# zkonduit/ezkl

Measured on NVIDIA H100. Metric: prove_time_s, lower is better.
Workload: dtype u32 limbs (254-bit Montgomery integers mod BN254 r/p)

## Files before the change

### ezkl_b200/csrc/debug.cu

```cuda
#include "../../include/ezkl_b200.h"
#include <cfenv>
#include <vector>
#include "msm.cuh"
#include "../../tools/experiments/fd.cuh"
#include "../../tools/experiments/msm_affine.cuh"

namespace b200 {
template <class Tag>
__global__ void k_dbg_field(int op, const Fp<Tag>* a, const Fp<Tag>* b, Fp<Tag>* o, size_t n) {
    size_t i = (size_t)blockIdx.x * blockDim.x + threadIdx.x;
    if (i >= n) return;
    Fp<Tag> x = fp_load(a + i), y = fp_load(b + i), r;
    if (op == 0) r = x + y; else if (op == 1) r = x - y; else if (op == 2) r = x * y; else if (op == 3) r = fp_inv(x); else r = fp_from_mont(x);
    fp_store(o + i, r);
}
__global__ void k_dbg_g1(int op, const G1Affine* a, const G1Affine* b, G1Affine* o, size_t n) {
    size_t i = (size_t)blockIdx.x * blockDim.x + threadIdx.x;
    if (i >= n) return;
    G1Affine p = a[i], q = b[i];
    G1Xyzz r;
    if (op == 0) r = g1_add_mixed(g1_to_xyzz(p), q);
    else if (op == 1) r = g1_dbl(g1_to_xyzz(p));
    else if (op == 2) r = g1_mul_small(g1_to_xyzz(p), q.x.l[0]);
    else if (op == 3) r = g1_add(g1_to_xyzz(p), g1_dbl_affine(q));
// ... 165 lines not shown
    for (size_t i = 0; i < n_ents; ++i) if ((ents[i] & 0x7fffffffu) + 1 > n_pts) n_pts = (ents[i] & 0x7fffffffu) + 1;
    tab.resize(n_pts);
    memcpy(tab.data(), table, 64 * n_pts);
    int rc = b200::msm_affine_host_chunks(tab.data(), ents, n_ents, chunk_start, chunk_len, nchunks, res.data());
    memcpy(out, res.data(), 64 * nchunks);
    return rc;
}
int b200_debug_bench(int variant, int iters, int blocks, int threads, float* ms) {
    Fq* d; B200_CUDA(cudaMalloc(&d, sizeof(Fq) * (size_t)blocks * threads));
    cudaEvent_t e0, e1; cudaEventCreate(&e0); cudaEventCreate(&e1);
    for (int rep = 0; rep < 2; ++rep) {
        cudaEventRecord(e0);
        switch (variant) {
            case 0: k_bench_mul<0><<<blocks, threads>>>(d, iters); break;
            case 1: k_bench_mul<1><<<blocks, threads>>>(d, iters); break;
            case 2: k_bench_mul<2><<<blocks, threads>>>(d, iters); break;
            case 3: k_bench_mul<3><<<blocks, threads>>>(d, iters); break;
            case 10: k_bench_hybrid<0><<<blocks, threads>>>(d, iters); break;
            case 11: k_bench_hybrid<1><<<blocks, threads>>>(d, iters); break;
            case 12: k_bench_hybrid<2><<<blocks, threads>>>(d, iters); break;
            case 13: k_bench_hybrid<3><<<blocks, threads>>>(d, iters); break;
            case 14: k_bench_hybrid<4><<<blocks, threads>>>(d, iters); break;
            case 15: k_bench_hybrid<5><<<blocks, threads>>>(d, iters); break;
            case 16: k_bench_hybrid<6><<<blocks, threads>>>(d, iters); break;
            case 17: k_bench_hybrid<7><<<blocks, threads>>>(d, iters); break;
            case 18: k_bench_hybrid<8><<<blocks, threads>>>(d, iters); break;
            default: k_bench_mul<4><<<blocks, threads>>>(d, iters); break;
        }
        cudaEventRecord(e1);
        B200_CUDA(cudaEventSynchronize(e1));
    }
    B200_CUDA(cudaEventElapsedTime(ms, e0, e1));
    cudaFree(d); cudaEventDestroy(e0); cudaEventDestroy(e1);
    return 0;
}
int b200_debug_bench_pipe(int variant, int iters, int blocks, int threads, float* ms) {
    uint64_t* d; B200_CUDA(cudaMalloc(&d, 8 * (size_t)blocks * threads));
    cudaEvent_t e0, e1; cudaEventCreate(&e0); cudaEventCreate(&e1);
    for (int rep = 0; rep < 2; ++rep) {
        cudaEventRecord(e0);
        switch (variant) {
            case 0: k_bench_pipe<0><<<blocks, threads>>>(d, iters); break;
            case 1: k_bench_pipe<1><<<blocks, threads>>>(d, iters); break;
            case 2: k_bench_pipe<2><<<blocks, threads>>>(d, iters); break;
            default: k_bench_pipe<3><<<blocks, threads>>>(d, iters); break;
        }
        cudaEventRecord(e1);
        B200_CUDA(cudaEventSynchronize(e1));
    }
    B200_CUDA(cudaEventElapsedTime(ms, e0, e1));
    cudaFree(d); cudaEventDestroy(e0); cudaEventDestroy(e1);
    return 0;
}
int b200_debug_digits_host(const b200_fr* s_canonical, size_t n, int c, int32_t* out) {
    const int W = (255 + c - 1) / c;
    for (size_t i = 0; i < n; ++i) {
        uint32_t v[8]; memcpy(v, &s_canonical[i], 32);
        uint32_t carry = 0;
        for (int w = 0; w < W; ++w) out[i * W + w] = msm_next_digit(v, c, &carry);
    }
    return 0;
}
int b200_debug_digit_slots_host(const b200_fr* s_canonical, size_t n, int c, int wpl, int32_t* out) {
    const int W = (255 + c - 1) / c;
    for (size_t i = 0; i < n; ++i) {
        uint32_t v[8]; memcpy(v, &s_canonical[i], 32);
        uint32_t carry = 0;
        MsmWindowSlot slot;
        for (int w = 0; w < W; ++w) {
            const int32_t d = msm_next_digit(v, c, &carry);
            int32_t* o = out + ((size_t)i * W + w) * 4;
            o[0] = (int32_t)slot.level; o[1] = slot.r;
            o[2] = d ? (int32_t)(slot.set_off + (uint32_t)(d < 0 ? -d : d) - 1u) : -1;
            o[3] = d < 0 ? -1 : (d > 0 ? 1 : 0);
            slot.next(c, wpl);
        }
    }
    return 0;
}
int b200_debug_msm_pick_levels(size_t n, int c, size_t max_table_bytes, int* s, int* L) {
    msm_pick_levels(n, c, max_table_bytes, s, L);
    return 0;
}
int b200_debug_host_g1_op(int op, const b200_g1_affine* a, const b200_g1_affine* b, b200_g1_affine* out, size_t n) {
    for (size_t i = 0; i < n; ++i) {
        G1Affine p, q; memcpy(&p, &a[i], 64); memcpy(&q, &b[i], 64);
        G1Xyzz r;
        if (op == 0) r = g1_add_mixed(g1_to_xyzz(p), q);
        else if (op == 1) r = g1_dbl(g1_to_xyzz(p));
        else if (op == 2) r = g1_mul_small(g1_to_xyzz(p), q.x.l[0]);
        else if (op == 3) r = g1_add(g1_to_xyzz(p), g1_dbl_affine(q));
        else r = g1_add_mixed(g1_to_xyzz(p), g1_neg(p));
        G1Affine o = g1_to_affine(r); memcpy(&out[i], &o, 64);
    }
    return 0;
}
int b200_debug_host_field_op(int field, int op, const b200_fr* a, const b200_fr* b, b200_fr* out, size_t n) {
    for (size_t i = 0; i < n; ++i) {
        if (field == 0) { Fr x, y, r; memcpy(&x, &a[i], 32); memcpy(&y, &b[i], 32);
            if (op == 0) r = x + y; else if (op == 1) r = x - y; else if (op == 2) r = x * y; else if (op == 3) r = fp_inv(x); else r = fp_from_mont(x);
            memcpy(&out[i], &r, 32);
        } else { Fq x, y, r; memcpy(&x, &a[i], 32); memcpy(&y, &b[i], 32);
            if (op == 0) r = x + y; else if (op == 1) r = x - y; else if (op == 2) r = x * y; else if (op == 3) r = fp_inv(x); else r = fp_from_mont(x);
            memcpy(&out[i], &r, 32);
        }
    }
    return 0;
}
}
#pragma GCC visibility pop
```

### ezkl_b200/csrc/msm.cu

```cuda
#include "msm.cuh"
#include "ec_coop.cuh"

namespace b200 {

static constexpr int HEAVY_CHUNKS = 32;
static constexpr int REDUCE_M_MAX = 32;
static constexpr int TREE_THREADS = 256;

int msm_default_window(size_t n) {
    int k = 0;
    while (((size_t)1 << (k + 1)) <= n) ++k;
    int c = k <= 10 ? 8 : (k <= 13 ? k - 2 : (k <= 17 ? k - 1 : (k <= 19 ? 17 : (k <= 21 ? 18 : 20))));
    if (c < 4) c = 4;
    if (c > 22) c = 22;
    return c;
}

__global__ void __launch_bounds__(128) k_table_next_level(const G1Affine* __restrict__ prev, G1Affine* __restrict__ next, size_t n, int c) {
    size_t i = (size_t)blockIdx.x * blockDim.x + threadIdx.x;
    if (i >= n) return;
    G1Affine p = prev[i];
    G1Xyzz a = g1_dbl_affine(p);
#pragma unroll 1
    for (int j = 1; j < c; ++j) a = g1_dbl(a);
    next[i] = g1_to_affine(a);
}

int msm_table_alloc(MsmTable* t, size_t n, int c, size_t max_table_bytes) {
    B200_CHECK(n > 0, -1, "msm_table_build: empty base vector");
    if (c <= 0) c = msm_default_window(n);
    int W = (255 + c - 1) / c, s = 1, L = W;
    msm_pick_levels(n, c, max_table_bytes, &s, &L);
    B200_CHECK((size_t)L * n < ((size_t)1 << 31), -1, "msm_table_build: L*n = %zu exceeds the 31-bit entry index", (size_t)L * n);
    t->n = n; t->c = c; t->W = W; t->s = s; t->L = L;
    B200_CUDA(cudaGetDevice(&t->device));
    const cudaError_t e = cudaMalloc(&t->d_table, t->bytes());
    if (e != cudaSuccess) {
        cudaGetLastError();
        t->d_table = nullptr;
        set_error("msm_table_build: %zu MiB table (%d levels of %zu points): %s", t->bytes() >> 20, L, n, cudaGetErrorString(e));
        return -2;
    }
    return 0;
}

int msm_table_build(MsmTable* t, const G1Affine* d_bases, cudaStream_t st) {
    const size_t n = t->n;
    if (d_bases) B200_CUDA(cudaMemcpyAsync(t->d_table, d_bases, sizeof(G1Affine) * n, cudaMemcpyDeviceToDevice, st));
    for (int j = 1; j < t->L; ++j) {
        k_table_next_level<<<div_up(n, 128), 128, 0, st>>>(t->d_table + (size_t)(j - 1) * n, t->d_table + (size_t)j * n, n, t->c * t->s); count_launch();
    }
    B200_CUDA(cudaGetLastError());
    return 0;
}
void msm_table_free(MsmTable* t) {
    if (t->d_table) cudaFree(t->d_table);
    t->d_table = nullptr;
}

template <bool SCATTER, bool SUBWIN>
__global__ void __launch_bounds__(256) k_digits(const Fr* __restrict__ scalars, size_t stride, uint32_t n, uint32_t table_n, uint32_t base_off, int c, int W,
                                                 uint32_t nbuckets, uint32_t* __restrict__ counters ,
                                                 const uint32_t* __restrict__ offs , uint32_t* __restrict__ ents, size_t ent_stride,
                                                 const uint32_t* __restrict__ skew, int wpl) {
    const uint32_t col = blockIdx.y;
    const bool aggregate = !SCATTER || skew[col] != 0;
    const Fr* sc = scalars + (size_t)col * stride;
    uint32_t* cnt = counters + (size_t)col * nbuckets;
    const uint32_t* off = SCATTER ? offs + (size_t)col * (nbuckets + 1) : nullptr;
    uint32_t* ent = SCATTER ? ents + (size_t)col * ent_stride : nullptr;
    const unsigned lane = threadIdx.x & 31;
    const uint32_t n_up = (n + 31u) & ~31u;
    for (uint32_t i = blockIdx.x * blockDim.x + threadIdx.x; i < n_up; i += gridDim.x * blockDim.x) {
        const bool valid = i < n;
        Fr s = fp_zero<FrTag>();
        if (valid) s = fp_from_mont(fp_load(sc + i));
        uint32_t carry = 0;
        MsmWindowSlot slot;
#pragma unroll 1
        for (int w = 0; w < W; ++w) {
            int32_t d = msm_next_digit(s.l, c, &carry);
            const uint32_t j = SUBWIN ? slot.level : (uint32_t)w;
            const bool nz = d != 0;
            const unsigned act = __ballot_sync(0xffffffffu, nz);
            if (nz && !aggregate) {
                const uint32_t bucket = (SUBWIN ? slot.set_off : 0u) + (uint32_t)(d < 0 ? -d : d) - 1u;
                ent[off[bucket] + atomicAdd(&cnt[bucket], 1u)] = (j * table_n + base_off + i) | (d < 0 ? 0x80000000u : 0u);
            } else if (nz) {
                const uint32_t bucket = (SUBWIN ? slot.set_off : 0u) + (uint32_t)(d < 0 ? -d : d) - 1u;
                const unsigned peers = __match_any_sync(act, bucket);
                const int leader = __ffs(peers) - 1;
                uint32_t base = 0;
                if ((int)lane == leader) base = atomicAdd(&cnt[bucket], (uint32_t)__popc(peers));
                if (SCATTER) {
                    base = __shfl_sync(peers, base, leader);
                    const uint32_t rank = __popc(peers & ((1u << lane) - 1u));
                    ent[off[bucket] + base + rank] = (j * table_n + base_off + i) | (d < 0 ? 0x80000000u : 0u);
                }
            }
            if (SUBWIN) slot.next(c, wpl);
        }
    }
}

__global__ void __launch_bounds__(1024) k_scan_buckets(const uint32_t* __restrict__ counts, uint32_t* __restrict__ offs, uint32_t* __restrict__ chunk_offs,
                                                        uint32_t nbuckets, uint32_t cap, uint32_t* __restrict__ skew ) {
    __shared__ uint32_t sh_max;
    if (threadIdx.x == 0) sh_max = 0;
    __syncthreads();
    const uint32_t col = blockIdx.x;
    const uint32_t lc = 31u - (uint32_t)__clz(cap);
    const uint32_t* cnt = counts + (size_t)col * nbuckets;
    uint32_t* off = offs + (size_t)col * (nbuckets + 1);
    uint32_t* coff = chunk_offs + (size_t)col * (nbuckets + 1);
    const uint32_t ipt = (nbuckets + blockDim.x - 1) / blockDim.x;
    const uint32_t lo = threadIdx.x * ipt, hi = min(lo + ipt, nbuckets);
    uint32_t s = 0, cs = 0;
    uint32_t mx = 0;
    const bool vec = (ipt & 3u) == 0 && lo + ipt <= nbuckets;
    if (vec) {
        const uint4* c4 = reinterpret_cast<const uint4*>(cnt + lo);
#pragma unroll 4
        for (uint32_t q = 0; q < (ipt >> 2); ++q) {
            const uint4 v = c4[q];
            s += v.x + v.y + v.z + v.w;
            cs += ((v.x + cap - 1) >> lc) + ((v.y + cap - 1) >> lc) + ((v.z + cap - 1) >> lc) + ((v.w + cap - 1) >> lc);
            mx = max(max(mx, v.x), max(max(v.y, v.z), v.w));
        }
    } else {
        for (uint32_t b = lo; b < hi; ++b) { uint32_t v = cnt[b]; s += v; cs += ((v + cap - 1) >> lc); mx = max(mx, v); }
    }
    if (mx) atomicMax(&sh_max, mx);
    uint32_t tot, ctot;
    uint32_t ex = block_exclusive_scan(s, &tot);
    uint32_t cex = block_exclusive_scan(cs, &ctot);
    if (vec) {
        const uint4* c4 = reinterpret_cast<const uint4*>(cnt + lo);
#pragma unroll 4
        for (uint32_t q = 0; q < (ipt >> 2); ++q) {
            const uint4 v = c4[q];
            const uint32_t b = lo + 4 * q;
            off[b] = ex; coff[b] = cex; ex += v.x; cex += ((v.x + cap - 1) >> lc);
            off[b + 1] = ex; coff[b + 1] = cex; ex += v.y; cex += ((v.y + cap - 1) >> lc);
            off[b + 2] = ex; coff[b + 2] = cex; ex += v.z; cex += ((v.z + cap - 1) >> lc);
            off[b + 3] = ex; coff[b + 3] = cex; ex += v.w; cex += ((v.w + cap - 1) >> lc);
        }
    } else {
        for (uint32_t b = lo; b < hi; ++b) { uint32_t v = cnt[b]; off[b] = ex; coff[b] = cex; ex += v; cex += ((v + cap - 1) >> lc); }
    }
    if (threadIdx.x == 0) {
        off[nbuckets] = tot; coff[nbuckets] = ctot;
        skew[col] = sh_max > 16u * (tot / nbuckets + 1u) ? 1u : 0u;
    }
}

__global__ void __launch_bounds__(256) k_fill_chunks(const uint32_t* __restrict__ offs, const uint32_t* __restrict__ chunk_offs, uint32_t nbuckets, uint32_t cap,
                                                      uint32_t* __restrict__ chunk_start, uint32_t* __restrict__ chunk_len, size_t chunk_stride,
                                                      uint32_t* __restrict__ len_hist , uint32_t* __restrict__ heavy , uint32_t heavy_stride) {
    extern __shared__ uint32_t sh_hist[];
    const uint32_t col = blockIdx.y;
    for (uint32_t j = threadIdx.x; j <= cap; j += blockDim.x) sh_hist[j] = 0;
    __syncthreads();
    const uint32_t* off = offs + (size_t)col * (nbuckets + 1);
    const uint32_t* coff = chunk_offs + (size_t)col * (nbuckets + 1);
    uint32_t* cs = chunk_start + (size_t)col * chunk_stride;
    uint32_t* cl = chunk_len + (size_t)col * chunk_stride;
    const uint32_t b = blockIdx.x * blockDim.x + threadIdx.x;
    if (b < nbuckets) {
        const uint32_t start = off[b], size = off[b + 1] - start, c0 = coff[b], nch = coff[b + 1] - c0;
        for (uint32_t j = 0; j < nch; ++j) {
            const uint32_t len = min(cap, size - j * cap);
            cs[c0 + j] = start + j * cap;
            cl[c0 + j] = len;
            if (j + 1 == nch) atomicAdd(&sh_hist[len], 1u);
        }
        if (nch > 1) atomicAdd(&sh_hist[cap], nch - 1);
        if (nch > (uint32_t)HEAVY_CHUNKS) {
            uint32_t* hv = heavy + (size_t)col * heavy_stride;
            uint32_t slot = atomicAdd(&hv[0], 1u);
            if (slot + 1 < heavy_stride) hv[1 + slot] = b;
        }
    }
    __syncthreads();
    uint32_t* gh = len_hist + (size_t)col * (cap + 1);
    for (uint32_t j = threadIdx.x; j <= cap; j += blockDim.x) if (sh_hist[j]) atomicAdd(&gh[j], sh_hist[j]);
}

__global__ void k_len_offsets(const uint32_t* __restrict__ len_hist, uint32_t* __restrict__ len_offs, uint32_t cap) {
    const uint32_t col = blockIdx.x;
    if (threadIdx.x != 0) return;
    const uint32_t* h = len_hist + (size_t)col * (cap + 1);
    uint32_t* o = len_offs + (size_t)col * (cap + 1);
    uint32_t acc = 0;
    for (int l = (int)cap; l >= 0; --l) { o[l] = acc; acc += h[l]; }
}

__global__ void __launch_bounds__(256) k_order_chunks(const uint32_t* __restrict__ chunk_len, size_t chunk_stride, const uint32_t* __restrict__ chunk_offs, uint32_t nbuckets,
                                                       const uint32_t* __restrict__ len_offs, uint32_t* __restrict__ len_cursor, uint32_t cap, uint32_t* __restrict__ order) {
    const uint32_t col = blockIdx.y;
    const uint32_t nchunks = chunk_offs[(size_t)col * (nbuckets + 1) + nbuckets];
    const uint32_t* cl = chunk_len + (size_t)col * chunk_stride;
    uint32_t* ord = order + (size_t)col * chunk_stride;
    const uint32_t* lo = len_offs + (size_t)col * (cap + 1);
    uint32_t* lc = len_cursor + (size_t)col * (cap + 1);
    const unsigned lane = threadIdx.x & 31;
    const uint32_t n_up = (nchunks + 31u) & ~31u;
    for (uint32_t i = blockIdx.x * blockDim.x + threadIdx.x; i < n_up; i += gridDim.x * blockDim.x) {
        const bool valid = i < nchunks;
        const uint32_t len = valid ? cl[i] : 0;
        const unsigned act = __ballot_sync(0xffffffffu, valid);
        if (valid) {
            const unsigned peers = __match_any_sync(act, len);
            const int leader = __ffs(peers) - 1;
            uint32_t base = 0;
            if ((int)lane == leader) base = atomicAdd(&lc[len], (uint32_t)__popc(peers));
            base = __shfl_sync(peers, base, leader);
            ord[lo[len] + base + __popc(peers & ((1u << lane) - 1u))] = i;
        }
    }
}

DEV G1Affine load_base(const G1Affine* __restrict__ table, uint32_t e) {
    const uint4* q = reinterpret_cast<const uint4*>(table + (e & 0x7fffffffu));
    uint4 a = __ldg(q), b = __ldg(q + 1), c = __ldg(q + 2), d = __ldg(q + 3);
    G1Affine p;
    p.x.l[0] = a.x; p.x.l[1] = a.y; p.x.l[2] = a.z; p.x.l[3] = a.w; p.x.l[4] = b.x; p.x.l[5] = b.y; p.x.l[6] = b.z; p.x.l[7] = b.w;
    p.y.l[0] = c.x; p.y.l[1] = c.y; p.y.l[2] = c.z; p.y.l[3] = c.w; p.y.l[4] = d.x; p.y.l[5] = d.y; p.y.l[6] = d.z; p.y.l[7] = d.w;
    return p;
}
__global__ void __launch_bounds__(128, 4) k_accumulate(const G1Affine* __restrict__ table, const uint32_t* __restrict__ ents, size_t ent_stride,
                                                        const uint32_t* __restrict__ chunk_start, const uint32_t* __restrict__ chunk_len, const uint32_t* __restrict__ order,
                                                        size_t chunk_stride, const uint32_t* __restrict__ chunk_offs, uint32_t nbuckets, G1Xyzz* __restrict__ chunk_sums) {
    const uint32_t col = blockIdx.y;
    const uint32_t nchunks = chunk_offs[(size_t)col * (nbuckets + 1) + nbuckets];
    const uint32_t* ent = ents + (size_t)col * ent_stride;
    for (uint32_t t = blockIdx.x * blockDim.x + threadIdx.x; t < nchunks; t += gridDim.x * blockDim.x) {
// ... 135 lines not shown
    acc = block_sum_coop(acc, sh);
    if (threadIdx.x == 0) out[col] = acc;
}

__global__ void __launch_bounds__(32) k_subwindow_fold(const G1Xyzz* __restrict__ set_sums , int s, int c, uint32_t batch, G1Xyzz* __restrict__ out) {
    const uint32_t col = blockIdx.x * blockDim.x + threadIdx.x;
    if (col >= batch) return;
    const G1Xyzz* rs = set_sums + (size_t)col * s;
    G1Xyzz acc = rs[s - 1];
#pragma unroll 1
    for (int r = s - 2; r >= 0; --r) {
#pragma unroll 1
        for (int k = 0; k < c; ++k) acc = g1_dbl(acc);
        acc = g1_add(acc, rs[r]);
    }
    out[col] = acc;
}

__global__ void __launch_bounds__(128) k_g1_generate(uint64_t seed, size_t n, G1Affine* __restrict__ out) {
    const size_t i = (size_t)blockIdx.x * blockDim.x + threadIdx.x;
    if (i >= n) return;
    uint32_t s[8];
    uint64_t z = seed + 0x9e3779b97f4a7c15ull * (uint64_t)(i + 1);
#pragma unroll
    for (int w = 0; w < 4; ++w) {
        z += 0x9e3779b97f4a7c15ull;
        uint64_t x = z; x = (x ^ (x >> 30)) * 0xbf58476d1ce4e5b9ull; x = (x ^ (x >> 27)) * 0x94d049bb133111ebull; x ^= x >> 31;
        s[2 * w] = (uint32_t)x; s[2 * w + 1] = (uint32_t)(x >> 32);
    }
    s[7] &= 0x0fffffffu;
    G1Affine g; g.x = fp_one<FqTag>(); g.y = fp_one<FqTag>() + fp_one<FqTag>();
    G1Xyzz acc = g1_xyzz_identity();
#pragma unroll 1
    for (int b = 251; b >= 0; --b) {
        acc = g1_dbl(acc);
        if ((s[b >> 5] >> (b & 31)) & 1) acc = g1_add_mixed(acc, g);
    }
    out[i] = g1_to_affine(acc);
}
int g1_generate_run(uint64_t seed, size_t n, G1Affine* d_out, cudaStream_t st) {
    if (n == 0) return 0;
    k_g1_generate<<<div_up(n, 128), 128, 0, st>>>(seed, n, d_out); count_launch();
    B200_CUDA(cudaGetLastError());
    return 0;
}

__global__ void __launch_bounds__(128) k_g1_fixed_base_mul(const Fr* __restrict__ scalars, size_t n, G1Affine base, G1Affine* __restrict__ out) {
    const size_t i = (size_t)blockIdx.x * blockDim.x + threadIdx.x;
    if (i >= n) return;
    const Fr s = fp_from_mont(fp_load(scalars + i));
    G1Xyzz acc = g1_xyzz_identity();
#pragma unroll 1
    for (int b = 253; b >= 0; --b) {
        acc = g1_dbl(acc);
        if ((s.l[b >> 5] >> (b & 31)) & 1) acc = g1_add_mixed(acc, base);
    }
    out[i] = g1_to_affine(acc);
}
int g1_fixed_base_mul_run(const Fr* d_scalars, size_t n, const G1Affine& base, G1Affine* d_out, cudaStream_t st) {
    if (n == 0) return 0;
    k_g1_fixed_base_mul<<<div_up(n, 128), 128, 0, st>>>(d_scalars, n, base, d_out); count_launch();
    B200_CUDA(cudaGetLastError());
    return 0;
}

int g1_sum_run(const G1Xyzz* d_points, size_t groups, size_t count, G1Xyzz* d_out, cudaStream_t st) {
    if (groups == 0) return 0;
    B200_CHECK(groups <= 0x7fffffffu && count <= 0xffffffffu, -1, "g1_sum: sizes out of range");
    k_final_coop<<<(unsigned)groups, TREE_THREADS, 0, st>>>(d_points, (uint32_t)count, d_out); count_launch();
    B200_CUDA(cudaGetLastError());
    return 0;
}

static uint32_t pick_cap(size_t total_entries) {
    size_t target = total_entries / ((size_t)sm_count() * 512 * 4);
    uint32_t cap = 16;
    while (cap < 512 && cap < target) cap <<= 1;
    return cap;
}

size_t msm_workspace_per_column(const MsmTable& t, size_t n) {
    const size_t nb = (size_t)t.s << (t.c - 1), ents = n * t.W;
    const size_t chunk_stride = nb + ents / 16 + 1;
    return ents * 4 + chunk_stride * (12 + sizeof(G1Xyzz)) + nb * (sizeof(G1Xyzz) + 24) + 65536 * (size_t)t.s;
}

int msm_run(const MsmTable& t, const Fr* d_scalars, size_t n, size_t stride, int batch, G1Xyzz* d_out, MsmWorkspace& ws, cudaStream_t st, size_t base_off) {
    B200_CHECK(base_off + n <= t.n, -1, "msm: pairs [%zu, %zu) but only %zu bases registered", base_off, base_off + n, t.n);
    B200_CHECK(batch > 0 && batch <= 65535, -1, "msm: batch %d out of range", batch);
    if (n == 0) {
        B200_CUDA(cudaMemsetAsync(d_out, 0, sizeof(G1Xyzz) * batch, st));
        return 0;
    }
    const int c = t.c, W = t.W, s = t.s;
    B200_CHECK((size_t)batch * s <= 65535, -1, "msm: batch %d x %d bucket sets out of range", batch, s);
    const uint32_t half = 1u << (c - 1), nb = half * (uint32_t)s;
    const int vcols = batch * s;
    const size_t ent_stride = (size_t)n * W;
    B200_CHECK(ent_stride < ((size_t)1 << 32), -1, "msm: n*W too large");
    const Config& cfg = config();
    const uint32_t cap = pick_cap(ent_stride * batch);
    const size_t chunk_stride = (size_t)nb + ent_stride / cap + 1;
    const uint32_t heavy_stride = (uint32_t)(ent_stride / ((size_t)cap * HEAVY_CHUNKS)) + 2;
    const size_t all_buckets = (size_t)batch * nb;
    uint32_t reduce_m = REDUCE_M_MAX, reduce_threads = TREE_THREADS;
    if (all_buckets <= ((size_t)1 << 15)) { reduce_m = 4; reduce_threads = 128; }
    else if (all_buckets <= ((size_t)1 << 18)) { reduce_m = 8; reduce_threads = 128; }
    else if (all_buckets <= ((size_t)5 << 17)) { reduce_m = 16; reduce_threads = 256; }
    else if (all_buckets < ((size_t)37 << 15)) { reduce_m = 32; reduce_threads = 128; }
    while (reduce_m > 1 && reduce_m > half) reduce_m >>= 1;
    if (cfg.msm_reduce_m >= 1 && cfg.msm_reduce_m <= 4096) reduce_m = (uint32_t)cfg.msm_reduce_m;
    if (cfg.msm_reduce_threads == 32 || cfg.msm_reduce_threads == 64 || cfg.msm_reduce_threads == 128 || cfg.msm_reduce_threads == 256) reduce_threads = (uint32_t)cfg.msm_reduce_threads;
    const bool coop = cfg.msm_reduce2 == 2 && all_buckets <= COOP_MAX_BUCKETS;
    if (coop) { reduce_m = cfg.msm_reduce_m >= 1 ? reduce_m : 8; reduce_threads = TREE_THREADS; }
    const uint32_t nparts = div_up(div_up(half, reduce_m), coop ? COOP_LT : reduce_threads);
    uint32_t final_threads = 32;
    while (final_threads < (uint32_t)TREE_THREADS && final_threads < nparts) final_threads <<= 1;

    const size_t n_hist = (size_t)batch * nb, n_len = (size_t)batch * (cap + 1), n_heavy = (size_t)batch * heavy_stride;
    const size_t counts_words = 2 * n_hist + 2 * n_len + n_heavy;
    if (ws.counts.ensure(counts_words * 4)) return -2;
    uint32_t* hist = ws.counts.as<uint32_t>();
    uint32_t* cursor = hist + n_hist;
    uint32_t* len_hist = cursor + n_hist;
    uint32_t* len_cursor = len_hist + n_len;
    uint32_t* heavy = len_cursor + n_len;
    const size_t n_off = (size_t)batch * (nb + 1);
    if (ws.offs.ensure((2 * n_off + n_len + (size_t)batch) * 4)) return -2;
    uint32_t* offs = ws.offs.as<uint32_t>();
    uint32_t* chunk_offs = offs + n_off;
    uint32_t* len_offs = chunk_offs + n_off;
    uint32_t* skew = len_offs + n_len;
    if (ws.ents.ensure((size_t)batch * ent_stride * 4)) return -2;
    uint32_t* ents = ws.ents.as<uint32_t>();
    if (ws.subs.ensure((size_t)batch * chunk_stride * 4 * 3)) return -2;
    uint32_t* chunk_start = ws.subs.as<uint32_t>();
    uint32_t* chunk_len = chunk_start + (size_t)batch * chunk_stride;
    uint32_t* order = chunk_len + (size_t)batch * chunk_stride;
    const size_t n_set = s > 1 ? (size_t)vcols : 0;
    if (ws.sums.ensure(sizeof(G1Xyzz) * ((size_t)batch * chunk_stride + (size_t)batch * nb + (size_t)vcols * nparts + n_set))) return -2;
    G1Xyzz* chunk_sums = ws.sums.as<G1Xyzz>();
    G1Xyzz* bucket_sums = chunk_sums + (size_t)batch * chunk_stride;
    G1Xyzz* partials = bucket_sums + (size_t)batch * nb;
    G1Xyzz* reduced = s > 1 ? partials + (size_t)vcols * nparts : d_out;

    ProfScope ps_total(PROF_MSM_TOTAL, st);
    B200_CUDA(cudaMemsetAsync(hist, 0, counts_words * 4, st));
    if (prof_enabled()) prof_mark(PROF_MSM_RECODE, st, true);
    const unsigned sms = (unsigned)sm_count();
    const unsigned dig_blocks = min(div_up(n, 256), sms * 8u);
    dim3 gd(dig_blocks, batch);
    if (s == 1) k_digits<false, false><<<gd, 256, 0, st>>>(d_scalars, stride, (uint32_t)n, (uint32_t)t.n, (uint32_t)base_off, c, W, nb, hist, nullptr, nullptr, 0, nullptr, 1);
    else k_digits<false, true><<<gd, 256, 0, st>>>(d_scalars, stride, (uint32_t)n, (uint32_t)t.n, (uint32_t)base_off, c, W, nb, hist, nullptr, nullptr, 0, nullptr, s);
    count_launch();
    {
        ProfScope ps(PROF_MSM_SCAN, st);
        k_scan_buckets<<<batch, 1024, 0, st>>>(hist, offs, chunk_offs, nb, cap, skew); count_launch();
    }
    if (s == 1) k_digits<true, false><<<gd, 256, 0, st>>>(d_scalars, stride, (uint32_t)n, (uint32_t)t.n, (uint32_t)base_off, c, W, nb, cursor, offs, ents, ent_stride, skew, 1);
    else k_digits<true, true><<<gd, 256, 0, st>>>(d_scalars, stride, (uint32_t)n, (uint32_t)t.n, (uint32_t)base_off, c, W, nb, cursor, offs, ents, ent_stride, skew, s);
    count_launch();
    k_fill_chunks<<<dim3(div_up(nb, 256), batch), 256, (cap + 1) * 4, st>>>(offs, chunk_offs, nb, cap, chunk_start, chunk_len, chunk_stride, len_hist, heavy, heavy_stride); count_launch();
    k_len_offsets<<<batch, 32, 0, st>>>(len_hist, len_offs, cap); count_launch();
    const unsigned ch_blocks = min(div_up(chunk_stride, 256), sms * 8u);
    k_order_chunks<<<dim3(ch_blocks, batch), 256, 0, st>>>(chunk_len, chunk_stride, chunk_offs, nb, len_offs, len_cursor, cap, order); count_launch();
    if (prof_enabled()) prof_mark(PROF_MSM_RECODE, st, false);
    const unsigned acc_blocks = min(div_up(chunk_stride, 128), sms * 16u);
    {
        ProfScope ps(PROF_MSM_ACCUMULATE, st);
        k_accumulate<<<dim3(acc_blocks, batch), 128, 0, st>>>(t.d_table, ents, ent_stride, chunk_start, chunk_len, order, chunk_stride, chunk_offs, nb, chunk_sums); count_launch();
    }
    ProfScope ps_tail(PROF_MSM_TAIL, st);
    k_combine<<<dim3(div_up(nb, 128), batch), 128, 0, st>>>(chunk_offs, nb, chunk_sums, chunk_stride, bucket_sums); count_launch();
    k_combine_heavy<<<dim3(32, batch), TREE_THREADS, 0, st>>>(heavy, heavy_stride, chunk_offs, nb, chunk_sums, chunk_stride, bucket_sums); count_launch();
    {
        ProfScope ps(PROF_MSM_REDUCE, st);
        if (coop) {
            k_reduce_coop<<<dim3(nparts, vcols), TREE_THREADS, 0, st>>>(bucket_sums, half, partials, nparts, reduce_m); count_launch();
            k_final_coop<<<vcols, TREE_THREADS, 0, st>>>(partials, nparts, reduced); count_launch();
        } else {
            k_reduce<1><<<dim3(nparts, vcols), reduce_threads, 0, st>>>(bucket_sums, half, partials, nparts, reduce_m); count_launch();
            k_final<<<vcols, final_threads, 0, st>>>(partials, nparts, reduced); count_launch();
        }
    }
    if (s > 1) {
        ProfScope ps(PROF_MSM_FOLD, st);
        k_subwindow_fold<<<div_up((size_t)batch, 32), 32, 0, st>>>(reduced, s, c, (uint32_t)batch, d_out); count_launch();
    }
    B200_CUDA(cudaGetLastError());
    return 0;
}

}
```

### ezkl_b200/csrc/msm.cuh

```cuda
#pragma once
#include "common.cuh"
#include "ec.cuh"

namespace b200 {

struct MsmTable {
    G1Affine* d_table = nullptr;
    size_t n = 0;
    int c = 0;
    int W = 0;
    int s = 1;
    int L = 0;
    int device = 0;
    size_t bytes() const { return sizeof(G1Affine) * n * (size_t)L; }
};

struct MsmWorkspace {
    DevBuf counts, offs, ents, subs, sums, misc;
};

int msm_default_window(size_t n);
inline void msm_pick_levels(size_t n, int c, size_t max_table_bytes, int* s, int* L) {
    const int W = (255 + c - 1) / c;
    const size_t level_bytes = sizeof(G1Affine) * n;
    for (int k = 1; k <= W; ++k) {
        const int l = (W + k - 1) / k;
        if (k == W || (size_t)l * level_bytes <= max_table_bytes) { *s = k; *L = l; return; }
    }
}
int msm_table_alloc(MsmTable* t, size_t n, int c, size_t max_table_bytes);
int msm_table_build(MsmTable* t, const G1Affine* d_bases, cudaStream_t st);
void msm_table_free(MsmTable* t);
int msm_run(const MsmTable& t, const Fr* d_scalars, size_t n, size_t stride, int batch, G1Xyzz* d_out,
            MsmWorkspace& ws, cudaStream_t st, size_t base_off = 0);
int g1_fixed_base_mul_run(const Fr* d_scalars, size_t n, const G1Affine& base, G1Affine* d_out, cudaStream_t st);
int g1_fft_run(const G1Affine* d_in, uint32_t log_n, const Fr& omega, const Fr* scale, G1Affine* d_out, DevBuf& scratch, cudaStream_t st);
int g1_generate_run(uint64_t seed, size_t n, G1Affine* d_out, cudaStream_t st);
int g1_sum_run(const G1Xyzz* d_points, size_t groups, size_t count, G1Xyzz* d_out, cudaStream_t st);
size_t msm_workspace_per_column(const MsmTable& t, size_t n);

HD int32_t msm_next_digit(uint32_t s[8], int c, uint32_t* carry) {
    uint32_t v = (s[0] & ((1u << c) - 1u)) + *carry;
#pragma unroll
    for (int j = 0; j < 7; ++j) s[j] = (s[j] >> c) | (s[j + 1] << (32 - c));
    s[7] >>= c;
    if (v > (1u << (c - 1))) { *carry = 1; return (int32_t)v - (int32_t)(1u << c); }
    *carry = 0;
    return (int32_t)v;
}

struct MsmWindowSlot {
    uint32_t level = 0, set_off = 0;
    int r = 0;
    HD void next(int c, int wpl) {
        set_off += 1u << (c - 1);
        if (++r == wpl) { r = 0; set_off = 0; ++level; }
    }
};

}
```

Baseline: 0.08885.

## Replace atomic bucket scatter with two-level shared-memory partitioned radix sort in MSM recode

Replaces the count/scan/scatter recode, which did global atomics per bucket, with a two-level radix sort. Digits are first partitioned into coarse partitions using shared-memory histograms per tile, staged and scattered in order. Each partition is then sorted into fine buckets in shared memory, and oversized partitions are split across several blocks with a separate histogram and scan. The goal is to cut global atomic contention and uncoalesced scattered writes. In exchange it adds several kernel launches, an extra uint2 intermediate buffer aliased onto the sums workspace, and a second digit walk per scalar.

```diff
diff --git a/ezkl_b200/csrc/debug.cu b/ezkl_b200/csrc/debug.cu
--- a/ezkl_b200/csrc/debug.cu
+++ b/ezkl_b200/csrc/debug.cu
@@ -271,6 +271,11 @@
     msm_pick_levels(n, c, max_table_bytes, s, L);
     return 0;
 }
+int b200_debug_msm_pick_recode(size_t n, int c, int s, uint32_t* out) {
+    const MsmRecodePlan r = msm_pick_recode(n, c, s);
+    out[0] = r.P; out[1] = (uint32_t)r.f; out[2] = r.T; out[3] = r.tiles;
+    return 0;
+}
 int b200_debug_host_g1_op(int op, const b200_g1_affine* a, const b200_g1_affine* b, b200_g1_affine* out, size_t n) {
     for (size_t i = 0; i < n; ++i) {
         G1Affine p, q; memcpy(&p, &a[i], 64); memcpy(&q, &b[i], 64);
diff --git a/ezkl_b200/csrc/msm.cu b/ezkl_b200/csrc/msm.cu
--- a/ezkl_b200/csrc/msm.cu
+++ b/ezkl_b200/csrc/msm.cu
@@ -58,100 +58,265 @@
     t->d_table = nullptr;
 }
 
-template <bool SCATTER, bool SUBWIN>
-__global__ void __launch_bounds__(256) k_digits(const Fr* __restrict__ scalars, size_t stride, uint32_t n, uint32_t table_n, uint32_t base_off, int c, int W,
-                                                 uint32_t nbuckets, uint32_t* __restrict__ counters ,
-                                                 const uint32_t* __restrict__ offs , uint32_t* __restrict__ ents, size_t ent_stride,
-                                                 const uint32_t* __restrict__ skew, int wpl) {
-    const uint32_t col = blockIdx.y;
-    const bool aggregate = !SCATTER || skew[col] != 0;
+DEV uint32_t smem_claim(uint32_t* sh, uint32_t key, unsigned act) {
+    const int first = __ffs(act) - 1;
+    if (__all_sync(act, key == __shfl_sync(act, key, first))) {
+        const unsigned lane = threadIdx.x & 31;
+        uint32_t base = 0;
+        if ((int)lane == first) base = atomicAdd(&sh[key], (uint32_t)__popc(act));
+        return __shfl_sync(act, base, first) + (uint32_t)__popc(act & ((1u << lane) - 1u));
+    }
+    return atomicAdd(&sh[key], 1u);
+}
+
+template <bool SUBWIN, class Fn>
+DEV void walk_digits(Fr s, uint32_t i, uint32_t table_n, uint32_t base_off, int c, int W, int wpl, Fn fn) {
+    uint32_t carry = 0;
+    MsmWindowSlot slot;
+#pragma unroll 1
+    for (int w = 0; w < W; ++w) {
+        const int32_t d = msm_next_digit(s.l, c, &carry);
+        const unsigned act = __ballot_sync(0xffffffffu, d != 0);
+        if (d != 0) {
+            const uint32_t j = SUBWIN ? slot.level : (uint32_t)w;
+            const uint32_t id = (SUBWIN ? slot.set_off : 0u) + (uint32_t)(d < 0 ? -d : d) - 1u;
+            fn(act, id, (j * table_n + base_off + i) | (d < 0 ? 0x80000000u : 0u));
+        }
+        if (SUBWIN) slot.next(c, wpl);
+    }
+}
+
+template <bool SUBWIN>
+__global__ void __launch_bounds__(256) k_part_count(const Fr* __restrict__ scalars, size_t stride, uint32_t n, uint32_t T, int c, int W, int wpl,
+                                                     int f, uint32_t P, uint32_t* __restrict__ cells ) {
+    extern __shared__ uint32_t sh_part[];
+    for (uint32_t p = threadIdx.x; p < P; p += blockDim.x) sh_part[p] = 0;
+    __syncthreads();
+    const Fr* sc = scalars + (size_t)blockIdx.y * stride;
+    const uint32_t lo = blockIdx.x * T, hi = min(lo + T, n);
+    for (uint32_t i = lo + threadIdx.x; i - threadIdx.x < hi; i += blockDim.x) {
+        const Fr s = i < hi ? fp_from_mont(fp_load(sc + i)) : fp_zero<FrTag>();
+        walk_digits<SUBWIN>(s, i, 0, 0, c, W, wpl, [&](unsigned act, uint32_t id, uint32_t) { smem_claim(sh_part, id >> f, act); });
+    }
+    __syncthreads();
+    const uint32_t tiles = gridDim.x;
+    uint32_t* out = cells + (size_t)blockIdx.y * ((size_t)P * tiles + 1);
+    for (uint32_t p = threadIdx.x; p < P; p += blockDim.x) out[(size_t)p * tiles + blockIdx.x] = sh_part[p];
+}
+
+static constexpr uint32_t PART_SPLIT = 65536;
+DEV uint32_t part_blocks(uint32_t len) { return len > PART_SPLIT ? (len + PART_SPLIT - 1) / PART_SPLIT : 0u; }
+DEV uint32_t block_partition(const uint32_t* mb, uint32_t P, uint32_t w) {
+    uint32_t lo = 0, hi = P;
+    while (hi - lo > 1) {
+        const uint32_t mid = (lo + hi) >> 1;
+        if (mb[mid] <= w) lo = mid; else hi = mid;
+    }
+    return lo;
+}
+
+__global__ void __launch_bounds__(1024) k_part_scan(uint32_t* __restrict__ cells, uint32_t P, uint32_t tiles, uint32_t* __restrict__ offs, uint32_t nb,
+                                                     uint32_t* __restrict__ mblk) {
+    const uint32_t col = blockIdx.x, m = P * tiles;
+    uint32_t* v = cells + (size_t)col * (m + 1);
+    const uint32_t ipt = (m + blockDim.x - 1) / blockDim.x;
+    const uint32_t lo = min(threadIdx.x * ipt, m), hi = min(lo + ipt, m);
+    uint32_t s = 0;
+#pragma unroll 8
+    for (uint32_t j = lo; j < hi; ++j) s += v[j];
+    uint32_t tot;
+    uint32_t ex = block_exclusive_scan(s, &tot);
+#pragma unroll 8
+    for (uint32_t j = lo; j < hi; ++j) { const uint32_t x = v[j]; v[j] = ex; ex += x; }
+    if (threadIdx.x == 0) { v[m] = tot; offs[(size_t)col * (nb + 1) + nb] = tot; }
+    __syncthreads();
+    uint32_t* mb = mblk + (size_t)col * (P + 1);
+    const uint32_t qpt = (P + blockDim.x - 1) / blockDim.x;
+    const uint32_t qlo = min(threadIdx.x * qpt, P), qhi = min(qlo + qpt, P);
+    uint32_t nblk = 0;
+    for (uint32_t p = qlo; p < qhi; ++p) nblk += part_blocks(v[(size_t)(p + 1) * tiles] - v[(size_t)p * tiles]);
+    uint32_t mtot;
+    uint32_t mex = block_exclusive_scan(nblk, &mtot);
+    for (uint32_t p = qlo; p < qhi; ++p) { mb[p] = mex; mex += part_blocks(v[(size_t)(p + 1) * tiles] - v[(size_t)p * tiles]); }
+    if (threadIdx.x == 0) mb[P] = mtot;
+}
+
+template <bool SUBWIN>
+__global__ void __launch_bounds__(256) k_part_scatter(const Fr* __restrict__ scalars, size_t stride, uint32_t n, uint32_t T, uint32_t table_n, uint32_t base_off,
+                                                       int c, int W, int wpl, int f, uint32_t P, const uint32_t* __restrict__ cells,
+                                                       uint2* __restrict__ part, size_t ent_stride) {
+    extern __shared__ uint32_t sh_part[];
+    uint32_t* cursor = sh_part;
+    uint32_t* cnt = cursor + P;
+    uint32_t* locs = cnt + P;
+    uint2* stage = reinterpret_cast<uint2*>(locs + P + (P & 1u));
+    const uint32_t tiles = gridDim.x, col = blockIdx.y;
+    const uint32_t* base = cells + (size_t)col * ((size_t)P * tiles + 1);
+    const uint32_t ipt = (P + blockDim.x - 1) / blockDim.x;
+    const uint32_t plo = min(threadIdx.x * ipt, P), phi = min(plo + ipt, P);
+    for (uint32_t p = plo; p < phi; ++p) cursor[p] = base[(size_t)p * tiles + blockIdx.x];
+    uint2* pt = part + (size_t)col * ent_stride;
     const Fr* sc = scalars + (size_t)col * stride;
-    uint32_t* cnt = counters + (size_t)col * nbuckets;
-    const uint32_t* off = SCATTER ? offs + (size_t)col * (nbuckets + 1) : nullptr;
-    uint32_t* ent = SCATTER ? ents + (size_t)col * ent_stride : nullptr;
-    const unsigned lane = threadIdx.x & 31;
-    const uint32_t n_up = (n + 31u) & ~31u;
-    for (uint32_t i = blockIdx.x * blockDim.x + threadIdx.x; i < n_up; i += gridDim.x * blockDim.x) {
-        const bool valid = i < n;
-        Fr s = fp_zero<FrTag>();
-        if (valid) s = fp_from_mont(fp_load(sc + i));
-        uint32_t carry = 0;
-        MsmWindowSlot slot;
-#pragma unroll 1
-        for (int w = 0; w < W; ++w) {
-            int32_t d = msm_next_digit(s.l, c, &carry);
-            const uint32_t j = SUBWIN ? slot.level : (uint32_t)w;
-            const bool nz = d != 0;
-            const unsigned act = __ballot_sync(0xffffffffu, nz);
-            if (nz && !aggregate) {
-                const uint32_t bucket = (SUBWIN ? slot.set_off : 0u) + (uint32_t)(d < 0 ? -d : d) - 1u;
-                ent[off[bucket] + atomicAdd(&cnt[bucket], 1u)] = (j * table_n + base_off + i) | (d < 0 ? 0x80000000u : 0u);
-            } else if (nz) {
-                const uint32_t bucket = (SUBWIN ? slot.set_off : 0u) + (uint32_t)(d < 0 ? -d : d) - 1u;
-                const unsigned peers = __match_any_sync(act, bucket);
-                const int leader = __ffs(peers) - 1;
-                uint32_t base = 0;
-                if ((int)lane == leader) base = atomicAdd(&cnt[bucket], (uint32_t)__popc(peers));
-                if (SCATTER) {
-                    base = __shfl_sync(peers, base, leader);
-                    const uint32_t rank = __popc(peers & ((1u << lane) - 1u));
-                    ent[off[bucket] + base + rank] = (j * table_n + base_off + i) | (d < 0 ? 0x80000000u : 0u);
-                }
+    const uint32_t fmask = (1u << f) - 1u;
+    const uint32_t lo = blockIdx.x * T, hi = min(lo + T, n);
+    for (uint32_t r0 = lo; r0 < hi; r0 += blockDim.x) {
+        for (uint32_t p = plo; p < phi; ++p) cnt[p] = 0;
+        __syncthreads();
+        const uint32_t i = r0 + threadIdx.x;
+        const Fr s = i < hi ? fp_from_mont(fp_load(sc + i)) : fp_zero<FrTag>();
+        walk_digits<SUBWIN>(s, i, 0, 0, c, W, wpl, [&](unsigned act, uint32_t id, uint32_t) { smem_claim(cnt, id >> f, act); });
+        __syncthreads();
+        uint32_t sum = 0;
+        for (uint32_t p = plo; p < phi; ++p) sum += cnt[p];
+        uint32_t tot;
+        uint32_t ex = block_exclusive_scan(sum, &tot);
+        for (uint32_t p = plo; p < phi; ++p) { const uint32_t x = cnt[p]; cnt[p] = ex; locs[p] = ex; ex += x; }
+        __syncthreads();
+        walk_digits<SUBWIN>(s, i, table_n, base_off, c, W, wpl, [&](unsigned act, uint32_t id, uint32_t e) {
+            const uint32_t p = id >> f;
+            stage[smem_claim(cnt, p, act)] = make_uint2(e, (p << 16) | (id & fmask));
+        });
+        __syncthreads();
+        for (uint32_t j = threadIdx.x; j < tot; j += blockDim.x) {
+            const uint2 v = stage[j];
+            const uint32_t p = v.y >> 16;
+            pt[cursor[p] + j - locs[p]] = make_uint2(v.x, v.y & 0xffffu);
+        }
+        __syncthreads();
+        for (uint32_t p = plo; p < phi; ++p) cursor[p] += cnt[p] - locs[p];
+    }
+}
+
+__global__ void __launch_bounds__(1024) k_part_block_hist(const uint32_t* __restrict__ cells, uint32_t P, uint32_t tiles, const uint32_t* __restrict__ mblk,
+                                                           const uint2* __restrict__ part, size_t ent_stride, int f, uint32_t* __restrict__ bh) {
+    extern __shared__ uint32_t sh_fine[];
+    const uint32_t col = blockIdx.y, w = blockIdx.x, B = 1u << f;
+    const uint32_t* mb = mblk + (size_t)col * (P + 1);
+    if (w >= mb[P]) return;
+    const uint32_t p = block_partition(mb, P, w);
+    const uint32_t* cl = cells + (size_t)col * ((size_t)P * tiles + 1);
+    const uint32_t lo = cl[(size_t)p * tiles] + (w - mb[p]) * PART_SPLIT, hi = min(lo + PART_SPLIT, cl[(size_t)(p + 1) * tiles]);
+    const uint2* pt = part + (size_t)col * ent_stride;
+    for (uint32_t b = threadIdx.x; b < B; b += blockDim.x) sh_fine[b] = 0;
+    __syncthreads();
+    for (uint32_t i = lo + threadIdx.x; i - threadIdx.x < hi; i += blockDim.x) {
+        const bool valid = i < hi;
+        const unsigned act = __ballot_sync(0xffffffffu, valid);
+        if (valid) smem_claim(sh_fine, pt[i].y, act);
+    }
+    __syncthreads();
+    uint32_t* out = bh + ((size_t)gridDim.x * col + w) * B;
+    for (uint32_t b = threadIdx.x; b < B; b += blockDim.x) out[b] = sh_fine[b];
+}
+__global__ void __launch_bounds__(1024) k_part_block_scan(const uint32_t* __restrict__ cells, uint32_t tiles, const uint32_t* __restrict__ mblk, uint32_t mmax,
+                                                           int f, uint32_t nb, uint32_t* __restrict__ bh, uint32_t* __restrict__ offs) {
+    const uint32_t p = blockIdx.x, P = gridDim.x, col = blockIdx.y, B = 1u << f;
+    const uint32_t* mb = mblk + (size_t)col * (P + 1);
+    const uint32_t nblk = mb[p + 1] - mb[p];
+    if (nblk == 0) return;
+    const uint32_t start = cells[(size_t)col * ((size_t)P * tiles + 1) + (size_t)p * tiles];
+    uint32_t* h = bh + ((size_t)mmax * col + mb[p]) * B;
+    const uint32_t ipt = (B + blockDim.x - 1) / blockDim.x;
+    const uint32_t lo = min(threadIdx.x * ipt, B), hi = min(lo + ipt, B);
+    uint32_t s = 0;
+    for (uint32_t b = lo; b < hi; ++b)
+        for (uint32_t k = 0; k < nblk; ++k) s += h[(size_t)k * B + b];
+    uint32_t tot;
+    uint32_t run = start + block_exclusive_scan(s, &tot);
+    uint32_t* off = offs + (size_t)col * (nb + 1);
+    for (uint32_t b = lo; b < hi; ++b) {
+        if ((p << f) + b < nb) off[(p << f) + b] = run;
+        for (uint32_t k = 0; k < nblk; ++k) { const uint32_t x = h[(size_t)k * B + b]; h[(size_t)k * B + b] = run; run += x; }
+    }
+}
+
+static constexpr uint32_t SORT_STAGE = 24576;
+__global__ void __launch_bounds__(1024) k_part_sort(const uint32_t* __restrict__ cells, uint32_t P, uint32_t tiles, const uint32_t* __restrict__ mblk,
+                                                     const uint32_t* __restrict__ bh, uint32_t mmax, const uint2* __restrict__ part, size_t ent_stride,
+                                                     int f, uint32_t nb, uint32_t* __restrict__ ents, uint32_t* __restrict__ offs) {
+    extern __shared__ uint32_t sh_fine[];
+    uint32_t* stage = sh_fine + (1u << f);
+    const uint32_t col = blockIdx.y, B = 1u << f;
+    const uint32_t* cl = cells + (size_t)col * ((size_t)P * tiles + 1);
+    if (blockIdx.x >= P) {
+        const uint32_t w = blockIdx.x - P;
+        const uint32_t* mb = mblk + (size_t)col * (P + 1);
+        if (w >= mb[P]) return;
+        const uint32_t q = block_partition(mb, P, w);
+        const uint32_t lo = cl[(size_t)q * tiles] + (w - mb[q]) * PART_SPLIT, hi = min(lo + PART_SPLIT, cl[(size_t)(q + 1) * tiles]);
+        const uint32_t* cur = bh + ((size_t)mmax * col + w) * B;
+        for (uint32_t b = threadIdx.x; b < B; b += blockDim.x) sh_fine[b] = cur[b];
+        __syncthreads();
+        const uint2* pt = part + (size_t)col * ent_stride;
+        uint32_t* ent = ents + (size_t)col * ent_stride;
+        for (uint32_t i = lo + threadIdx.x; i - threadIdx.x < hi; i += blockDim.x) {
+            const bool valid = i < hi;
+            const unsigned act = __ballot_sync(0xffffffffu, valid);
+            if (valid) {
+                const uint2 v = pt[i];
+                ent[smem_claim(sh_fine, v.y, act)] = v.x;
             }
-            if (SUBWIN) slot.next(c, wpl);
-        }
-    }
-}
-
-__global__ void __launch_bounds__(1024) k_scan_buckets(const uint32_t* __restrict__ counts, uint32_t* __restrict__ offs, uint32_t* __restrict__ chunk_offs,
-                                                        uint32_t nbuckets, uint32_t cap, uint32_t* __restrict__ skew ) {
-    __shared__ uint32_t sh_max;
-    if (threadIdx.x == 0) sh_max = 0;
-    __syncthreads();
+        }
+        return;
+    }
+    const uint32_t p = blockIdx.x;
+    const uint32_t start = cl[(size_t)p * tiles], len = cl[(size_t)(p + 1) * tiles] - start;
+    if (len > PART_SPLIT) return;
+    const uint32_t len_up = (len + 31u) & ~31u;
+    const uint2* pt = part + (size_t)col * ent_stride + start;
+    uint32_t* ent = ents + (size_t)col * ent_stride + start;
+    for (uint32_t b = threadIdx.x; b < B; b += blockDim.x) sh_fine[b] = 0;
+    __syncthreads();
+    for (uint32_t i = threadIdx.x; i < len_up; i += blockDim.x) {
+        const bool valid = i < len;
+        const unsigned act = __ballot_sync(0xffffffffu, valid);
+        if (valid) smem_claim(sh_fine, pt[i].y, act);
+    }
+    __syncthreads();
+    const uint32_t ipt = (B + blockDim.x - 1) / blockDim.x;
+    const uint32_t lo = min(threadIdx.x * ipt, B), hi = min(lo + ipt, B);
+    uint32_t s = 0;
+    for (uint32_t b = lo; b < hi; ++b) s += sh_fine[b];
+    uint32_t tot;
+    uint32_t ex = block_exclusive_scan(s, &tot);
+    uint32_t* off = offs + (size_t)col * (nb + 1);
+    for (uint32_t b = lo; b < hi; ++b) {
+        const uint32_t x = sh_fine[b];
+        sh_fine[b] = ex;
+        if ((p << f) + b < nb) off[(p << f) + b] = start + ex;
+        ex += x;
+    }
+    __syncthreads();
+    uint32_t* dst = len <= SORT_STAGE ? stage : ent;
+    for (uint32_t i = threadIdx.x; i < len_up; i += blockDim.x) {
+        const bool valid = i < len;
+        const unsigned act = __ballot_sync(0xffffffffu, valid);
+        if (valid) {
+            const uint2 v = pt[i];
+            dst[smem_claim(sh_fine, v.y, act)] = v.x;
+        }
+    }
+    if (len <= SORT_STAGE) {
+        __syncthreads();
+        for (uint32_t i = threadIdx.x; i < len; i += blockDim.x) ent[i] = stage[i];
+    }
+}
+
+__global__ void __launch_bounds__(1024) k_scan_chunks(const uint32_t* __restrict__ offs, uint32_t* __restrict__ chunk_offs, uint32_t nbuckets, uint32_t cap) {
     const uint32_t col = blockIdx.x;
     const uint32_t lc = 31u - (uint32_t)__clz(cap);
-    const uint32_t* cnt = counts + (size_t)col * nbuckets;
-    uint32_t* off = offs + (size_t)col * (nbuckets + 1);
+    const uint32_t* off = offs + (size_t)col * (nbuckets + 1);
     uint32_t* coff = chunk_offs + (size_t)col * (nbuckets + 1);
     const uint32_t ipt = (nbuckets + blockDim.x - 1) / blockDim.x;
-    const uint32_t lo = threadIdx.x * ipt, hi = min(lo + ipt, nbuckets);
-    uint32_t s = 0, cs = 0;
-    uint32_t mx = 0;
-    const bool vec = (ipt & 3u) == 0 && lo + ipt <= nbuckets;
-    if (vec) {
-        const uint4* c4 = reinterpret_cast<const uint4*>(cnt + lo);
-#pragma unroll 4
-        for (uint32_t q = 0; q < (ipt >> 2); ++q) {
-            const uint4 v = c4[q];
-            s += v.x + v.y + v.z + v.w;
-            cs += ((v.x + cap - 1) >> lc) + ((v.y + cap - 1) >> lc) + ((v.z + cap - 1) >> lc) + ((v.w + cap - 1) >> lc);
-            mx = max(max(mx, v.x), max(max(v.y, v.z), v.w));
-        }
-    } else {
-        for (uint32_t b = lo; b < hi; ++b) { uint32_t v = cnt[b]; s += v; cs += ((v + cap - 1) >> lc); mx = max(mx, v); }
-    }
-    if (mx) atomicMax(&sh_max, mx);
-    uint32_t tot, ctot;
-    uint32_t ex = block_exclusive_scan(s, &tot);
+    const uint32_t lo = min(threadIdx.x * ipt, nbuckets), hi = min(lo + ipt, nbuckets);
+    uint32_t cs = 0;
+#pragma unroll 8
+    for (uint32_t b = lo; b < hi; ++b) cs += (off[b + 1] - off[b] + cap - 1) >> lc;
+    uint32_t ctot;
     uint32_t cex = block_exclusive_scan(cs, &ctot);
-    if (vec) {
-        const uint4* c4 = reinterpret_cast<const uint4*>(cnt + lo);
-#pragma unroll 4
-        for (uint32_t q = 0; q < (ipt >> 2); ++q) {
-            const uint4 v = c4[q];
-            const uint32_t b = lo + 4 * q;
-            off[b] = ex; coff[b] = cex; ex += v.x; cex += ((v.x + cap - 1) >> lc);
-            off[b + 1] = ex; coff[b + 1] = cex; ex += v.y; cex += ((v.y + cap - 1) >> lc);
-            off[b + 2] = ex; coff[b + 2] = cex; ex += v.z; cex += ((v.z + cap - 1) >> lc);
-            off[b + 3] = ex; coff[b + 3] = cex; ex += v.w; cex += ((v.w + cap - 1) >> lc);
-        }
-    } else {
-        for (uint32_t b = lo; b < hi; ++b) { uint32_t v = cnt[b]; off[b] = ex; coff[b] = cex; ex += v; cex += ((v + cap - 1) >> lc); }
-    }
-    if (threadIdx.x == 0) {
-        off[nbuckets] = tot; coff[nbuckets] = ctot;
-        skew[col] = sh_max > 16u * (tot / nbuckets + 1u) ? 1u : 0u;
-    }
+#pragma unroll 8
+    for (uint32_t b = lo; b < hi; ++b) { coff[b] = cex; cex += (off[b + 1] - off[b] + cap - 1) >> lc; }
+    if (threadIdx.x == 0) coff[nbuckets] = ctot;
 }
 
 __global__ void __launch_bounds__(256) k_fill_chunks(const uint32_t* __restrict__ offs, const uint32_t* __restrict__ chunk_offs, uint32_t nbuckets, uint32_t cap,
@@ -453,7 +618,9 @@
 size_t msm_workspace_per_column(const MsmTable& t, size_t n) {
     const size_t nb = (size_t)t.s << (t.c - 1), ents = n * t.W;
     const size_t chunk_stride = nb + ents / 16 + 1;
-    return ents * 4 + chunk_stride * (12 + sizeof(G1Xyzz)) + nb * (sizeof(G1Xyzz) + 24) + 65536 * (size_t)t.s;
+    const MsmRecodePlan rp = msm_pick_recode(n, t.c, t.s);
+    const size_t cells = (size_t)rp.P * rp.tiles + 1 + rp.P + 1 + ((2 * ents / PART_SPLIT) << rp.f);
+    return ents * 4 + chunk_stride * (12 + sizeof(G1Xyzz)) + nb * (sizeof(G1Xyzz) + 16) + cells * 4 + 65536 * (size_t)t.s;
 }
 
 int msm_run(const MsmTable& t, const Fr* d_scalars, size_t n, size_t stride, int batch, G1Xyzz* d_out, MsmWorkspace& ws, cudaStream_t st, size_t base_off) {
@@ -488,20 +655,24 @@
     uint32_t final_threads = 32;
     while (final_threads < (uint32_t)TREE_THREADS && final_threads < nparts) final_threads <<= 1;
 
-    const size_t n_hist = (size_t)batch * nb, n_len = (size_t)batch * (cap + 1), n_heavy = (size_t)batch * heavy_stride;
-    const size_t counts_words = 2 * n_hist + 2 * n_len + n_heavy;
-    if (ws.counts.ensure(counts_words * 4)) return -2;
-    uint32_t* hist = ws.counts.as<uint32_t>();
-    uint32_t* cursor = hist + n_hist;
-    uint32_t* len_hist = cursor + n_hist;
+    const MsmRecodePlan rp = msm_pick_recode(n, c, s);
+    const uint32_t m_cells = rp.P * rp.tiles;
+    const uint32_t mmax = (uint32_t)(2 * ent_stride / PART_SPLIT);
+    const size_t n_len = (size_t)batch * (cap + 1), n_heavy = (size_t)batch * heavy_stride;
+    const size_t zeroed_words = 2 * n_len + n_heavy;
+    const size_t n_cells = (size_t)batch * (m_cells + 1), n_mblk = (size_t)batch * (rp.P + 1), n_bh = (size_t)batch * mmax << rp.f;
+    if (ws.counts.ensure((zeroed_words + n_cells + n_mblk + n_bh) * 4)) return -2;
+    uint32_t* len_hist = ws.counts.as<uint32_t>();
     uint32_t* len_cursor = len_hist + n_len;
     uint32_t* heavy = len_cursor + n_len;
+    uint32_t* cells = heavy + n_heavy;
+    uint32_t* mblk = cells + n_cells;
+    uint32_t* bh = mblk + n_mblk;
     const size_t n_off = (size_t)batch * (nb + 1);
-    if (ws.offs.ensure((2 * n_off + n_len + (size_t)batch) * 4)) return -2;
+    if (ws.offs.ensure((2 * n_off + n_len) * 4)) return -2;
     uint32_t* offs = ws.offs.as<uint32_t>();
     uint32_t* chunk_offs = offs + n_off;
     uint32_t* len_offs = chunk_offs + n_off;
-    uint32_t* skew = len_offs + n_len;
     if (ws.ents.ensure((size_t)batch * ent_stride * 4)) return -2;
     uint32_t* ents = ws.ents.as<uint32_t>();
     if (ws.subs.ensure((size_t)batch * chunk_stride * 4 * 3)) return -2;
@@ -509,28 +680,43 @@
     uint32_t* chunk_len = chunk_start + (size_t)batch * chunk_stride;
     uint32_t* order = chunk_len + (size_t)batch * chunk_stride;
     const size_t n_set = s > 1 ? (size_t)vcols : 0;
-    if (ws.sums.ensure(sizeof(G1Xyzz) * ((size_t)batch * chunk_stride + (size_t)batch * nb + (size_t)vcols * nparts + n_set))) return -2;
+    const size_t sums_bytes = sizeof(G1Xyzz) * ((size_t)batch * chunk_stride + (size_t)batch * nb + (size_t)vcols * nparts + n_set);
+    if (ws.sums.ensure(std::max(sums_bytes, (size_t)batch * ent_stride * sizeof(uint2)))) return -2;
+    uint2* part = ws.sums.as<uint2>();
     G1Xyzz* chunk_sums = ws.sums.as<G1Xyzz>();
     G1Xyzz* bucket_sums = chunk_sums + (size_t)batch * chunk_stride;
     G1Xyzz* partials = bucket_sums + (size_t)batch * nb;
     G1Xyzz* reduced = s > 1 ? partials + (size_t)vcols * nparts : d_out;
 
     ProfScope ps_total(PROF_MSM_TOTAL, st);
-    B200_CUDA(cudaMemsetAsync(hist, 0, counts_words * 4, st));
+    B200_CUDA(cudaMemsetAsync(len_hist, 0, zeroed_words * 4, st));
     if (prof_enabled()) prof_mark(PROF_MSM_RECODE, st, true);
     const unsigned sms = (unsigned)sm_count();
-    const unsigned dig_blocks = min(div_up(n, 256), sms * 8u);
-    dim3 gd(dig_blocks, batch);
-    if (s == 1) k_digits<false, false><<<gd, 256, 0, st>>>(d_scalars, stride, (uint32_t)n, (uint32_t)t.n, (uint32_t)base_off, c, W, nb, hist, nullptr, nullptr, 0, nullptr, 1);
-    else k_digits<false, true><<<gd, 256, 0, st>>>(d_scalars, stride, (uint32_t)n, (uint32_t)t.n, (uint32_t)base_off, c, W, nb, hist, nullptr, nullptr, 0, nullptr, s);
+    const dim3 gt(rp.tiles, batch), gp(rp.P, batch);
+    const size_t sh_part = (size_t)rp.P * 4, sh_sort = ((size_t)4 << rp.f) + (size_t)SORT_STAGE * 4;
+    const size_t sh_scatter = ((size_t)3 * rp.P + (rp.P & 1u)) * 4 + (size_t)256 * W * sizeof(uint2);
+    B200_CUDA(cudaFuncSetAttribute(k_part_sort, cudaFuncAttributeMaxDynamicSharedMemorySize, (int)sh_sort));
+    B200_CUDA(cudaFuncSetAttribute(s == 1 ? k_part_scatter<false> : k_part_scatter<true>, cudaFuncAttributeMaxDynamicSharedMemorySize, (int)sh_scatter));
+    const uint32_t un = (uint32_t)n, tn = (uint32_t)t.n, bo = (uint32_t)base_off;
+    if (s == 1) k_part_count<false><<<gt, 256, sh_part, st>>>(d_scalars, stride, un, rp.T, c, W, 1, rp.f, rp.P, cells);
+    else k_part_count<true><<<gt, 256, sh_part, st>>>(d_scalars, stride, un, rp.T, c, W, s, rp.f, rp.P, cells);
     count_launch();
     {
         ProfScope ps(PROF_MSM_SCAN, st);
-        k_scan_buckets<<<batch, 1024, 0, st>>>(hist, offs, chunk_offs, nb, cap, skew); count_launch();
-    }
-    if (s == 1) k_digits<true, false><<<gd, 256, 0, st>>>(d_scalars, stride, (uint32_t)n, (uint32_t)t.n, (uint32_t)base_off, c, W, nb, cursor, offs, ents, ent_stride, skew, 1);
-    else k_digits<true, true><<<gd, 256, 0, st>>>(d_scalars, stride, (uint32_t)n, (uint32_t)t.n, (uint32_t)base_off, c, W, nb, cursor, offs, ents, ent_stride, skew, s);
+        k_part_scan<<<batch, 1024, 0, st>>>(cells, rp.P, rp.tiles, offs, nb, mblk); count_launch();
+    }
+    if (s == 1) k_part_scatter<false><<<gt, 256, sh_scatter, st>>>(d_scalars, stride, un, rp.T, tn, bo, c, W, 1, rp.f, rp.P, cells, part, ent_stride);
+    else k_part_scatter<true><<<gt, 256, sh_scatter, st>>>(d_scalars, stride, un, rp.T, tn, bo, c, W, s, rp.f, rp.P, cells, part, ent_stride);
     count_launch();
+    if (mmax > 0) {
+        k_part_block_hist<<<dim3(mmax, batch), 1024, (size_t)4 << rp.f, st>>>(cells, rp.P, rp.tiles, mblk, part, ent_stride, rp.f, bh); count_launch();
+        k_part_block_scan<<<gp, 1024, 0, st>>>(cells, rp.tiles, mblk, mmax, rp.f, nb, bh, offs); count_launch();
+    }
+    k_part_sort<<<dim3(rp.P + mmax, batch), 1024, sh_sort, st>>>(cells, rp.P, rp.tiles, mblk, bh, mmax, part, ent_stride, rp.f, nb, ents, offs); count_launch();
+    {
+        ProfScope ps(PROF_MSM_SCAN, st);
+        k_scan_chunks<<<batch, 1024, 0, st>>>(offs, chunk_offs, nb, cap); count_launch();
+    }
     k_fill_chunks<<<dim3(div_up(nb, 256), batch), 256, (cap + 1) * 4, st>>>(offs, chunk_offs, nb, cap, chunk_start, chunk_len, chunk_stride, len_hist, heavy, heavy_stride); count_launch();
     k_len_offsets<<<batch, 32, 0, st>>>(len_hist, len_offs, cap); count_launch();
     const unsigned ch_blocks = min(div_up(chunk_stride, 256), sms * 8u);
diff --git a/ezkl_b200/csrc/msm.cuh b/ezkl_b200/csrc/msm.cuh
--- a/ezkl_b200/csrc/msm.cuh
+++ b/ezkl_b200/csrc/msm.cuh
@@ -27,6 +27,23 @@
         const int l = (W + k - 1) / k;
         if (k == W || (size_t)l * level_bytes <= max_table_bytes) { *s = k; *L = l; return; }
     }
+}
+static constexpr uint32_t MSM_PART_MAX = 4096;
+struct MsmRecodePlan {
+    uint32_t P = 1;
+    int f = 8;
+    uint32_t T = 1024;
+    uint32_t tiles = 1;
+};
+inline MsmRecodePlan msm_pick_recode(size_t n, int c, int s) {
+    const int W = (255 + c - 1) / c;
+    const size_t nb = (size_t)s << (c - 1);
+    MsmRecodePlan r;
+    while (((nb + ((size_t)1 << r.f) - 1) >> r.f) > MSM_PART_MAX) ++r.f;
+    r.P = (uint32_t)((nb + ((size_t)1 << r.f) - 1) >> r.f);
+    while (r.T < 16384 && (size_t)r.T * W < (size_t)64 * r.P) r.T <<= 1;
+    r.tiles = (uint32_t)((n + r.T - 1) / r.T);
+    return r;
 }
 int msm_table_alloc(MsmTable* t, size_t n, int c, size_t max_table_bytes);
 int msm_table_build(MsmTable* t, const G1Affine* d_bases, cudaStream_t st);
```

New measurement: 0.08184 (median of 6 runs). 7.9% less time.
